# GreenleafLab/NucleoATAC

Measured on AMD Instinct MI355X. Metric: Mbp/s through occ+nuc signal pipeline, higher is better.
Workload: dtype f64

## Files before the change

nucleoatac_amd/csrc/natac_api.hip:

```cpp
#include "../../include/natac.h"
#ifndef NATAC_GNBL
#define NATAC_GNBL 2
#endif
#include "natac_kernels.hpp"
#include "natac_fft_bg.hpp"
#include "natac_occ_fast.hpp"
#include "natac_cand.hpp"
#include "natac_covsweep.hpp"
#include "natac_textz.hpp"
#include "natac_cores.hpp"
#include "natac_writer.hpp"
#include "natac_tabix.hpp"
#include "natac_pack.hpp"
#include "natac_bam.hpp"
#include "natac_bam_dev.hpp"
#include "natac_fragfile.hpp"
#include "natac_fragfile_dev.hpp"
#include "natac_fasta.hpp"
#include "natac_fuzzfit.hpp"
#include "natac_bedtab.hpp"
#include "natac_runtime.hpp"
#include "natac_pwmfit.hpp"
#include "natac_sites.hpp"
#include "natac_cellcounts.hpp"
// ... 138 lines not shown
template <int STEP>
static void occ_fast_launch(const OccFastLaunch &f) {
    natac_batch *b = f.b;
    occ_gsum_launch<STEP>(f);
    auto kd = (f.of.flags & 2) ? (f.rn16 ? natac_occ_decide<STEP, 16, true> : natac_occ_decide<STEP, 4, true>)
                               : (f.rn16 ? natac_occ_decide<STEP, 16, false> : natac_occ_decide<STEP, 4, false>);
    const bool heavy_first = b->ctx->occ_ordered;
    hipLaunchKernelGGL(kd, dim3((b->n_tiles_occ + (heavy_first ? HEAVY_CAP : 0) + 3) / 4), dim3(256), f.lds_od, b->ctx->stream, f.ct, b->d_tiles_occ,
                       b->n_tiles_occ, b->d_ranges_occ, heavy_first ? b->d_order_occ : nullptr, f.of, b->d_blk_off, b->total_blocks, b->d_gsum, b->d_grid[0], b->d_grid[1], b->d_grid[2], b->d_defer,
                       b->d_defer + 1);
}

extern "C" {

int natac_abi_version(void) { return NATAC_ABI_VERSION; }
const char *natac_last_error(void) { return g_err.c_str(); }

int natac_device_count(int *count) {
    if (!count) return fail(NATAC_E_ARG, "count is NULL");
    int n = 0;
    hipError_t e = hipGetDeviceCount(&n);
    if (e != hipSuccess) {
        *count = 0;
        return fail(NATAC_E_HIP, "hipGetDeviceCount: %s", hipGetErrorString(e));
    }
    *count = n;
    return NATAC_OK;
}

int natac_ctx_create(int device_id, natac_ctx **out) {
    if (!out) return fail(NATAC_E_ARG, "out is NULL");
    *out = nullptr;
    int n = 0;
    HIPCHK(hipGetDeviceCount(&n));
    if (device_id < 0 || device_id >= n) return fail(NATAC_E_ARG, "device %d out of range (%d devices)", device_id, n);
    HIPCHK(hipSetDevice(device_id));
    natac_ctx *c = new natac_ctx();
    c->device = device_id;
    HIPCHK(hipGetDeviceProperties(&c->prop, device_id));
    HIPCHK(hipStreamCreateWithFlags(&c->stream, hipStreamNonBlocking));
    HIPCHK(hipEventCreate(&c->t0));
    HIPCHK(hipEventCreate(&c->t1));
    {
        const char *e = getenv("NATAC_BG_DIRECT");
        c->bg_direct = e && e[0] == '1';
        e = getenv("NATAC_BG_EXT");
        c->bg_ext = !(e && e[0] == '0');
        e = getenv("NATAC_OCC_GENERAL");
        c->occ_force_general = e && e[0] == '1';
        e = getenv("NATAC_OCC_ORDER");
        c->occ_ordered = !(e && e[0] == '0');
        e = getenv("NATAC_SMOOTH_FUSED");
        c->smooth_fused = !(e && e[0] == '0');
    }
    *out = c;
    return NATAC_OK;
}

void natac_ctx_destroy(natac_ctx *c) {
    if (!c) return;
    (void)hipSetDevice(c->device);
    (void)sync_all(c);
    prof_collect(c);
    if (c->t0) (void)hipEventDestroy(c->t0);
    if (c->t1) (void)hipEventDestroy(c->t1);
    if (c->ck_stream) (void)hipStreamDestroy(c->ck_stream);
    if (c->ck_start) (void)hipEventDestroy(c->ck_start);
    if (c->d_ck) (void)hipFree(c->d_ck);
    if (c->copy_stream) (void)hipStreamDestroy(c->copy_stream);
    if (c->stream) (void)hipStreamDestroy(c->stream);
    delete c;
}

int natac_ctx_sync(natac_ctx *c) {
    if (!c) return fail(NATAC_E_ARG, "ctx is NULL");
    HIPCHK(hipSetDevice(c->device));
    HIPCHK(sync_all(c));
    prof_collect(c);
    return NATAC_OK;
}

int natac_ctx_device_info(natac_ctx *c, char *name, size_t name_len, int *n_cu, size_t *mem_bytes) {
    if (!c) return fail(NATAC_E_ARG, "ctx is NULL");
    if (name && name_len) {
        snprintf(name, name_len, "%s (%s)", c->prop.name, c->prop.gcnArchName);
    }
    if (n_cu) *n_cu = c->prop.multiProcessorCount;
    if (mem_bytes) *mem_bytes = c->prop.totalGlobalMem;
    return NATAC_OK;
}

int natac_ctx_device_ids(natac_ctx *c, int *hip_device, char *pci_bus_id, size_t pci_len) {
    if (!c) return fail(NATAC_E_ARG, "ctx is NULL");
    if (hip_device) *hip_device = c->device;
    if (pci_bus_id && pci_len) {
        pci_bus_id[0] = 0;
        HIPCHK(hipDeviceGetPCIBusId(pci_bus_id, (int)pci_len, c->device));
    }
    return NATAC_OK;
}

int natac_set_vmat(natac_ctx *c, const double *mat, int lower, int upper, int w) {
    if (!c || !mat) return fail(NATAC_E_ARG, "null argument");
    if (lower < 0 || upper <= lower || w < 0) return fail(NATAC_E_ARG, "bad vmat geometry lower=%d upper=%d w=%d", lower, upper, w);
    HIPCHK(hipSetDevice(c->device));
    HIPCHK(sync_all(c));
// ... 1126 lines not shown
    for (int64_t k = 0; k < n_cand; ++k) var[k] = var[k] * cov_reads(reads[(size_t)k]);
    return NATAC_OK;
}

static bool peaks_smooth_arm(const natac_batch *b, int order) {
    return order >= 1 && order <= 255 && peaks_plan(b->max_len, order).forms_smooth;
}

static int run_peaks_impl(natac_batch *b, const double *sig_a, const double *sig_b, bool with_stats, double min_signal, int sep,
                          int boundary, int order, const double *jitter, int64_t n_jitter, int64_t *n_cand, bool form_smooth = false) {
    if (!b || !jitter || !n_cand) return fail(NATAC_E_ARG, "null argument");
    natac_ctx *c = b->ctx;
    if (order < 1 || order > 255 || sep < 1 || boundary < 0) return fail(NATAC_E_ARG, "bad peak parameters");
    const int maxL = b->max_len;
    if (n_jitter < maxL) return fail(NATAC_E_ARG, "jitter stream (%lld) shorter than the longest chunk (%d)", (long long)n_jitter, maxL);
    HIPCHK(hipSetDevice(c->device));
    HIPCHK(sync_all(c));
    int rc;
    if (with_stats && (rc = ensure_srow(c))) return rc;
    if (!b->d_jitter || b->n_jitter < maxL) {
        if ((rc = dev_upload(c, b->d_jitter, jitter, (size_t)maxL))) return rc;
        HIPCHK(hipStreamSynchronize(c->stream));
        b->n_jitter = maxL;
    } else {
        HIPCHK(hipMemcpyAsync(b->d_jitter, jitter, (size_t)maxL * sizeof(double), hipMemcpyHostToDevice, c->stream));
        HIPCHK(hipStreamSynchronize(c->stream));
    }
    if (b->pk_order != order) {
        std::vector<long long> cap((size_t)b->nc + 1, 0);
        for (int i = 0; i < b->nc; ++i) cap[i + 1] = cap[i] + b->h_len[i] / (order + 1) + 2;
        b->slot_total = cap[b->nc];
        b->d_cap_off.reset(); b->d_slot.reset();
        if ((rc = dev_upload(c, b->d_cap_off, cap.data(), (size_t)b->nc + 1))) return rc;
        HIPCHK(hipStreamSynchronize(c->stream));
        if ((rc = dev_alloc(b->d_slot, (size_t)b->slot_total))) return rc;
        b->pk_order = order;
    }
    if (!b->d_pk_count && (rc = dev_alloc(b->d_pk_count, (size_t)b->nc))) return rc;
    if (!b->d_pk_offs && (rc = dev_alloc(b->d_pk_offs, (size_t)b->nc + 1))) return rc;
    if (form_smooth &&
        (rc = ensure_window(c, c->d_win_nuc, &c->win_nuc_M, &c->win_nuc_sd, b->out.smooth_M, b->out.smooth_sd, &c->win_nuc_sum))) return rc;
    const PeakPlan plan = peaks_plan(maxL, order);
    PeakSearch s{sig_a, sig_b, b->d_jitter, min_signal, boundary, order, sep, b->d_cap_off, b->d_slot, b->d_pk_count, b->d_status,
                 b->d_pk_offs, c->d_win_nuc, c->win_nuc_sum, form_smooth ? b->d_track[NATAC_T_SMOOTH].get() : nullptr};
    if (plan.global_lists) {
        if (b->d_pk_big.size() < (size_t)b->slot_total * 2 + 2 && (rc = dev_alloc(b->d_pk_big, (size_t)b->slot_total * 2 + 2))) return rc;
        s.big_sig = b->d_pk_big;
        s.big_pos = (int *)(b->d_pk_big + b->slot_total);
        s.big_state = (unsigned char *)(s.big_pos + b->slot_total);
    }
    natac_ctx::Ev ev;
    prof_begin(c, NATAC_K_CAND, ev);
    const ChunkTable ct = make_table(b);
    if ((rc = peaks_enqueue(plan, ct, b->nc, s, c->stream))) return rc;
    long long total = 0;
    HIPCHK(hipGetLastError());
    if (form_smooth) b->out.track[NATAC_T_SMOOTH] = TS_RUN;
    HIPCHK(hipMemcpyAsync(&total, b->d_pk_offs + b->nc, sizeof(long long), hipMemcpyDeviceToHost, c->stream));
    HIPCHK(hipStreamSynchronize(c->stream));
    if (total > b->pk_cap) {
        b->d_pk_chunk.reset(); b->d_pk_pos.reset(); b->d_pk_out.reset();
        b->pk_cap = 0;
        const long long cap = total + total / 4 + 16;
        if ((rc = dev_alloc(b->d_pk_chunk, (size_t)cap)) || (rc = dev_alloc(b->d_pk_pos, (size_t)cap)) ||
            (rc = dev_alloc(b->d_pk_out, (size_t)3 * cap))) {
            b->d_pk_chunk.reset(); b->d_pk_pos.reset();
            return rc;
        }
        b->pk_cap = cap;
    }
    if (total > 0) {
        hipLaunchKernelGGL(natac_compact_candidates, dim3((b->nc + 3) / 4), dim3(256), 0, c->stream, b->nc, b->d_pk_count, b->d_pk_offs,
                           b->d_cap_off, b->d_slot, b->d_pk_chunk, b->d_pk_pos);
        if (with_stats) {
            const VMatDev vm = make_vmat(c);
            launch_candidates(c, ct, vm, b->d_pk_chunk, b->d_pk_pos, total, b->d_track[NATAC_T_NUC_COV], b->d_track[NATAC_T_NORM],
                              b->out.bg_gen == c->model_gen ? b->d_bnum : nullptr, b->out.bg_gen == c->model_gen ? b->d_bcov : nullptr,
                              b->d_pk_out, b->d_pk_out + b->pk_cap, b->d_pk_out + 2 * b->pk_cap,
                              b->ranges256_w == c->vw ? b->d_tile256_first : nullptr, b->ranges256_w == c->vw ? b->d_ranges256 : nullptr);
        }
    }
    b->pk_has_stats = with_stats;
    prof_end(c, ev);
    HIPCHK(hipGetLastError());
    b->pk_n = total;
    *n_cand = total;
    return NATAC_OK;
}

int natac_peaks_plan(int32_t max_len, int32_t order, int32_t *kernel, int32_t *bt, int32_t *nj, int32_t *mask, int32_t *global_lists,
                     int32_t *forms_smooth, int32_t *pk_cap, int64_t *lds_bytes) {
    if (!kernel || !bt || !nj || !mask || !global_lists || !forms_smooth || !pk_cap || !lds_bytes) return fail(NATAC_E_ARG, "null argument");
    if (max_len < 1 || order < 1 || order > 255) return fail(NATAC_E_ARG, "natac_peaks_plan: a positive length and an order in 1..255");
    const PeakPlan p = peaks_plan(max_len, order);
    *kernel = p.kernel; *bt = p.bt; *nj = p.nj; *mask = p.mask; *global_lists = p.global_lists; *forms_smooth = p.forms_smooth;
    *pk_cap = p.pk_cap;
    lds_bytes[0] = (int64_t)p.lds; lds_bytes[1] = (int64_t)p.lds_smooth;
    return NATAC_OK;
}

int natac_run_peaks(natac_batch *b, double min_signal, int sep, int boundary, int order, const double *jitter, int64_t n_jitter,
                    int64_t *n_cand) {
    if (!b) return fail(NATAC_E_ARG, "batch is NULL");
    int rc;
    const bool form_smooth = b->out.track[NATAC_T_SMOOTH] == TS_PENDING && peaks_smooth_arm(b, order);
    if ((!form_smooth && (rc = need_track(b, NATAC_T_SMOOTH))) || (rc = need_candidate_inputs(b)) ||
        (rc = need_nuc_geometry(b, "natac_run_peaks"))) return rc;
// ... 201 lines not shown
```

nucleoatac_amd/csrc/natac_peaks.hpp:

```cpp
#pragma once
#include "natac_kernels.hpp"
#include "natac_runtime.hpp"

#include <utility>

namespace natac {

constexpr int PEAK_MAX = 2048;
constexpr int PK_SM_H = 30;

constexpr int PK_REG_MAX_NJ = 16;
constexpr int PK_REG1K_MIN_NJ = 256 * PK_REG_MAX_NJ / 1024 + 1;
constexpr int PK_REG_MAX_LDS = 150 * 1024;
constexpr int PK_SEG = 4096;
constexpr int PK_LIST_MIN = 2 * 128;

__host__ __device__ constexpr int peaks_list_cap(int maxL, int order) {
    const int m = maxL / (order + 1) + 2;
    return ((m < PEAK_MAX ? m : PEAK_MAX) + 7) & ~7;
}
__host__ __device__ constexpr int peaks_list_region(int pk_cap) { return pk_cap * (int)(sizeof(double) + sizeof(int) + 1); }
__host__ __device__ constexpr int peaks_wave_stride(int region, int nw) { return (region / nw) & ~7; }
__host__ __device__ constexpr bool peaks_masks_in_registers(int stride, int nj) { return stride < nj * 8; }
__host__ __device__ constexpr bool peaks_two_phase(int stride, int nj, int order) { return order > 2 && stride >= nj * 8 + PK_LIST_MIN; }
enum PeakKernel : int { PK_KERNEL_REG = 0, PK_KERNEL_SEG = 1 };
enum PeakMask : int { PK_MASK_NONE = -1, PK_MASK_REGISTERS = 0, PK_MASK_TWO_PHASE = 1, PK_MASK_DIRECT = 2 };
__host__ __device__ constexpr PeakMask peaks_mask_mode(int stride, int nj, int order) {
    return peaks_masks_in_registers(stride, nj) ? PK_MASK_REGISTERS : peaks_two_phase(stride, nj, order) ? PK_MASK_TWO_PHASE : PK_MASK_DIRECT;
}
__host__ __device__ constexpr int peaks_reg_ysn(int bt_nj, int order, bool smooth) {
    return (bt_nj + ((smooth && 2 * PK_SM_H > 2 * order + 1) ? 2 * PK_SM_H : 2 * order + 1)) & ~1;
}

struct PeakPlan {
    PeakKernel kernel;
    int bt, nj, pk_cap;
    PeakMask mask;
    bool global_lists;
    bool forms_smooth;
    size_t lds, lds_smooth;
};

__host__ __device__ constexpr PeakPlan peaks_plan(int maxL, int order) {
    PeakPlan p{};
    p.pk_cap = peaks_list_cap(maxL, order);
    const int region = peaks_list_region(p.pk_cap);
    p.bt = maxL <= 256 * PK_REG_MAX_NJ ? 256 : 1024;
    p.nj = (maxL - 1) / p.bt + 1;
    if (p.nj <= PK_REG_MAX_NJ) p.lds = (size_t)peaks_reg_ysn(p.bt * p.nj, order, false) * sizeof(double) + region;
    if (p.nj <= PK_REG_MAX_NJ && (p.bt == 256 || p.lds <= (size_t)PK_REG_MAX_LDS)) {
        p.kernel = PK_KERNEL_REG;
        p.mask = peaks_mask_mode(peaks_wave_stride(region, p.bt / 64), p.nj, order);
        p.forms_smooth = p.bt == 256 && p.mask != PK_MASK_REGISTERS;
        p.lds_smooth = p.forms_smooth ? (size_t)peaks_reg_ysn(p.bt * p.nj, order, true) * sizeof(double) + region : p.lds;
    } else {
        p.kernel = PK_KERNEL_SEG;
        p.bt = 256;
        p.nj = 0;
        p.mask = PK_MASK_NONE;
        p.global_lists = maxL / (order + 1) + 2 > p.pk_cap;
        p.lds = p.lds_smooth = (size_t)((PK_SEG + 2 * order + 1) & ~1) * sizeof(double) + region;
    }
    return p;
}
static_assert(peaks_plan(4096, 12).bt == 256 && peaks_plan(4096, 12).nj == PK_REG_MAX_NJ && peaks_plan(4096, 12).forms_smooth &&
              peaks_plan(4097, 12).bt == 1024 && peaks_plan(4097, 12).nj == PK_REG1K_MIN_NJ && !peaks_plan(4097, 12).forms_smooth &&
              peaks_plan(16384, 12).kernel == PK_KERNEL_REG && peaks_plan(16385, 12).kernel == PK_KERNEL_SEG &&
              peaks_plan(4096, 150).mask == PK_MASK_REGISTERS && !peaks_plan(4096, 150).forms_smooth, "peak search plan");

__device__ __forceinline__ void peaks_thin_and_write(int n, int pk_cap, int sep, const double *sig, const int *pos, unsigned char *state,
                                                      int *wave_cnt, int *__restrict__ dst, int *__restrict__ count_out,
                                                      int *__restrict__ status_out) {
    const int wave = threadIdx.x >> 6, lane = threadIdx.x & 63, bt = blockDim.x, nw = bt >> 6;
    const bool overflow = n > pk_cap;
    if (overflow) n = pk_cap;
    for (;;) {
        int nfree = 0;
        for (int i = threadIdx.x; i < n; i += bt) {
            if (state[i] != 0) continue;
            const double si = sig[i];
            const int pi = pos[i];
            bool top = true;
            for (int k = i - 1; top && k >= 0 && pi - pos[k] < sep; --k) top = !(state[k] <= 1 && sig[k] > si);
            for (int k = i + 1; top && k < n && pos[k] - pi < sep; ++k) top = !(state[k] <= 1 && sig[k] >= si);
            if (top) state[i] = 1; else ++nfree;
        }
        __syncthreads();
        for (int i = threadIdx.x; i < n; i += bt) {
            if (state[i] != 0) continue;
            const int pi = pos[i];
            bool ex = false;
            for (int k = i - 1; !ex && k >= 0 && pi - pos[k] < sep; --k) ex = state[k] == 1;
            for (int k = i + 1; !ex && k < n && pos[k] - pi < sep; ++k) ex = state[k] == 1;
            if (ex) { state[i] = 2; --nfree; }
        }
        if (__syncthreads_or(nfree > 0) == 0) break;
    }
    int m_out = 0;
    for (int base = 0; base < n; base += bt) {
        const int i = base + threadIdx.x;
        const bool kp = i < n && state[i] == 1;
        const unsigned long long m = __ballot(kp);
        if (lane == 0) wave_cnt[wave] = __popcll(m);
        __syncthreads();
        int off = m_out;
        int tot = 0;
        for (int w = 0; w < nw; ++w) { const int cw = wave_cnt[w]; off += (w < wave) ? cw : 0; tot += cw; }
        if (kp) dst[off + __popcll(m & ((1ull << lane) - 1ull))] = pos[i];
        m_out += tot;
        __syncthreads();
    }
    if (threadIdx.x == 0) {
        *count_out = m_out;
        if (overflow) atomicOr(status_out, 2);
    }
}

__global__ void __launch_bounds__(256) natac_peaks_chunk(ChunkTable ct, const double *__restrict__ norm,
                                                           const double *__restrict__ smooth, const double *__restrict__ jitter,
                                                           double min_signal, int boundary, int order, int sep, int seg, int pk_cap,
                                                           const long long *__restrict__ cap_off, int *__restrict__ cand_slot,
                                                           int *__restrict__ count, int *__restrict__ status,
                                                           double *__restrict__ big_sig, int *__restrict__ big_pos,
                                                           unsigned char *__restrict__ big_state) {
    extern __shared__ __attribute__((aligned(16))) double smem[];
    __shared__ double red[4];
    __shared__ int wave_cnt[16];
    __shared__ int row_cnt[4 * 16];
    const int ysn = (seg + 2 * order + 1) & ~1;
    double *ys = smem;
    double *sig = ys + ysn;
    int *pos = (int *)(sig + pk_cap);
    unsigned char *state = (unsigned char *)(pos + pk_cap);
    const int chunk = blockIdx.x;
    {
        const long long c0 = cap_off[chunk];
        const int cap_c = (int)(cap_off[chunk + 1] - c0);
        if (big_sig && cap_c > pk_cap) { sig = big_sig + c0; pos = big_pos + c0; state = big_state + c0; pk_cap = cap_c; }
    }
    const int L = ct.chunk_len[chunk];
    const long long ob = ct.out_off[chunk];
    const int wave = threadIdx.x >> 6, lane = threadIdx.x & 63;
    double mn = __builtin_inf();
    for (int g0 = threadIdx.x; g0 < L; g0 += 8 * 256) {
        double v[8];
#pragma unroll
        for (int q = 0; q < 8; ++q) {
            const int g = g0 + 256 * q;
            v[q] = __builtin_nan("");
            if (g < L) v[q] = smooth ? norm[ob + g] + smooth[ob + g] : norm[ob + g];
        }
#pragma unroll
        for (int q = 0; q < 8; ++q)
            if (v[q] == v[q]) mn = fmin(mn, v[q]);
    }
    mn = wave_min(mn);
    if (lane == 0) red[wave] = mn;
    __syncthreads();
    const double fillv = fmin(fmin(red[0], red[1]), fmin(red[2], red[3]));
    if (fillv == __builtin_inf()) {
        if (threadIdx.x == 0) count[chunk] = 0;
        return;
    }
    int n = 0;
    for (int x0 = 0; x0 < L; x0 += seg) {
        const int len = min(seg, L - x0);
        __syncthreads();
        for (int u0 = threadIdx.x; u0 < len + 2 * order; u0 += 8 * 256) {
            double v[8], jt[8];
#pragma unroll
            for (int q = 0; q < 8; ++q) {
                const int u = u0 + 256 * q;
                int g = x0 - order + u;
                g = g < 0 ? 0 : (g > L - 1 ? L - 1 : g);
                v[q] = smooth ? norm[ob + g] + smooth[ob + g] : norm[ob + g];
                jt[q] = jitter[g];
            }
#pragma unroll
            for (int q = 0; q < 8; ++q) {
                const int u = u0 + 256 * q;
                if (u < len + 2 * order) ys[u] = ((v[q] != v[q]) ? fillv : v[q]) * (1 + jt[q]);
            }
        }
        __syncthreads();
        unsigned pkf = 0;
#pragma unroll
        for (int it = 0; it < 16; ++it) {
            const int t = 256 * it + threadIdx.x;
            bool pk = t < len;
            if (pk) {
                const double y = ys[t + order];
                for (int sft = 1; sft <= order && pk; ++sft) pk = (y > ys[t + order + sft]) && (y > ys[t + order - sft]);
            }
            pkf |= pk ? (1u << it) : 0u;
        }
        double v[16];
#pragma unroll
        for (int it = 0; it < 16; ++it) {
            const int g = x0 + 256 * it + threadIdx.x;
            v[it] = 0.0;
            if (pkf & (1u << it)) v[it] = smooth ? norm[ob + g] + smooth[ob + g] : norm[ob + g];
        }
        unsigned long long bal[16];
#pragma unroll
        for (int it = 0; it < 16; ++it) {
            const int g = x0 + 256 * it + threadIdx.x;
            if (v[it] != v[it]) v[it] = fillv;
            const bool pk = (pkf & (1u << it)) && (v[it] >= min_signal) && (g >= boundary) && (g < L - boundary);
            bal[it] = __ballot(pk);
            if (lane == 0) row_cnt[it * 4 + wave] = __popcll(bal[it]);
        }
        __syncthreads();
#pragma unroll
        for (int it = 0; it < 16; ++it) {
            int off = n;
#pragma unroll
            for (int w = 0; w < 4; ++w) {
                const int cw = row_cnt[it * 4 + w];
                off += (w < wave) ? cw : 0;
                n += cw;
            }
            if ((bal[it] >> lane) & 1ull) {
                const int i = off + __popcll(bal[it] & ((1ull << lane) - 1ull));
                if (i < pk_cap) { pos[i] = x0 + 256 * it + threadIdx.x; sig[i] = v[it]; state[i] = 0; }
            }
        }
    }
    __syncthreads();
    peaks_thin_and_write(n, pk_cap, sep, sig, pos, state, wave_cnt, cand_slot + cap_off[chunk], count + chunk, status + chunk);
}

template <int NJ, int BT, bool SMOOTH = false>
__global__ void __launch_bounds__(BT) natac_peaks_chunk_reg(ChunkTable ct, const double *__restrict__ norm,
                                                               const double *__restrict__ smooth, const double *__restrict__ jitter,
                                                               double min_signal, int boundary, int order, int sep, int pk_cap,
                                                               const long long *__restrict__ cap_off, int *__restrict__ cand_slot,
                                                               int *__restrict__ count, int *__restrict__ status,
                                                               const double *__restrict__ win, double win_sum,
                                                               double *__restrict__ smooth_out) {
    extern __shared__ __attribute__((aligned(16))) double smem[];
    constexpr int NW = BT / 64;
    __shared__ double red[NW];
    __shared__ int wave_cnt[16];
    __shared__ int row_cnt[NW * NJ];
    const int ysn = peaks_reg_ysn(BT * NJ, order, SMOOTH);
    double *ys = smem;
    double *sig = ys + ysn;
    int *pos = (int *)(sig + pk_cap);
    unsigned char *state = (unsigned char *)(pos + pk_cap);
    const int chunk = blockIdx.x;
    const int L = ct.chunk_len[chunk];
    const long long ob = ct.out_off[chunk];
    const int wave = threadIdx.x >> 6, lane = threadIdx.x & 63;
    double v[NJ], jt[NJ];
    if constexpr (SMOOTH) {
        constexpr int H = PK_SM_H, M = 2 * H + 1;
        static_assert(BT >= 2 * H && M < 64, "the halo is zeroed by one pass of the workgroup; a window's validity bits fit one word");
        __shared__ unsigned long long okb[NW * NJ + 2];
        double *xs = smem;
#pragma unroll
        for (int j = 0; j < NJ; ++j) {
            const int g = threadIdx.x + BT * j;
            double x = __builtin_nan("");
            if (g < L) x = norm[ob + g];
            v[j] = x;
            const bool okv = x == x;
            xs[H + g] = okv ? (x < 0 ? 0.0 : x) : 0.0;
            const unsigned long long m = __ballot(okv);
            if (lane == 0) okb[1 + NW * j + wave] = m;
        }
        if (threadIdx.x < 2 * H) xs[threadIdx.x < H ? threadIdx.x : BT * NJ + threadIdx.x] = 0.0;
        if (threadIdx.x == 0) { okb[0] = 0ull; okb[NW * NJ + 1] = 0ull; }
        __syncthreads();
        const int g0 = threadIdx.x * NJ;
        double num[NJ];
#pragma unroll
        for (int o = 0; o < NJ; ++o) num[o] = 0.0;
        if (g0 < L) {
#pragma unroll
            for (int kk = 0; kk < 2 * H + NJ; ++kk) {
                const int k = 2 * H + NJ - 1 - kk;
                const double r = xs[g0 + k];
#pragma unroll
                for (int o = 0; o < NJ; ++o) {
                    const int n = o + 2 * H - k;
                    if (n >= 0 && n < M) num[o] = fma(win[n], r, num[o]);
                }
            }
        }
        __syncthreads();
        if (g0 < L) {
#pragma unroll
            for (int o = 0; o < NJ; ++o) xs[g0 + o] = num[o];
        }
        __syncthreads();
#pragma unroll
        for (int j = 0; j < NJ; ++j) {
            const int g = threadIdx.x + BT * j;
            const bool in = g < L;
            jt[j] = 0.0;
            if (in) jt[j] = jitter[g];
            double den = win_sum;
            const int iw = NW * j + wave;
            constexpr unsigned long long HM = (1ull << H) - 1ull;
            const bool clean = (okb[iw] >> (64 - H)) == HM && okb[iw + 1] == ~0ull && (okb[iw + 2] & HM) == HM;
            if (__ballot(!clean) != 0ull) {
                constexpr unsigned long long FULL = (1ull << M) - 1ull;
                const int p = g - H + 64, i = p >> 6, sh = p & 63;
                unsigned long long f = okb[i] >> sh;
                if (sh) f |= okb[i + 1] << (64 - sh);
                f &= FULL;
                bool generic = false;
                if (in && f != FULL) {
                    const int lo = __builtin_ctzll(f | (1ull << M)), hi = __builtin_clzll(f | 1ull) - (64 - M);
                    if (f == 0ull) den = 0.0;
                    else if (f == ((FULL >> lo) << lo)) den = win[M + 2 * H - lo];
                    else if (f == (FULL >> hi)) den = win[2 * M + hi];
                    else generic = true;
                }
                if (__ballot(generic) != 0ull) {
                    double d = 0.0;
#pragma unroll 8
                    for (int n = 0; n < M; ++n) {
                        const double wv = win[n];
                        if ((f >> (2 * H - n)) & 1ull) d = fma(wv, 1.0, d);
                    }
                    if (generic) den = d;
                }
            }
            if (in) {
                const double s = (den == 0.0) ? __builtin_nan("") : xs[g] / den;
                smooth_out[ob + g] = s;
                v[j] += s;
            }
        }
    } else {
#pragma unroll
    for (int j = 0; j < NJ; ++j) {
        const int g = threadIdx.x + BT * j;
        v[j] = __builtin_nan("");
        jt[j] = 0.0;
        if (g < L) {
            v[j] = smooth ? norm[ob + g] + smooth[ob + g] : norm[ob + g];
            jt[j] = jitter[g];
        }
    }
    }
    double mn = __builtin_inf();
#pragma unroll
    for (int j = 0; j < NJ; ++j)
        if (v[j] == v[j]) mn = fmin(mn, v[j]);
    mn = wave_min(mn);
    if (lane == 0) red[wave] = mn;
    __syncthreads();
    double fillv = red[0];
#pragma unroll
    for (int w = 1; w < NW; ++w) fillv = fmin(fillv, red[w]);
    if (fillv == __builtin_inf()) {
        if (threadIdx.x == 0) count[chunk] = 0;
        return;
    }
#pragma unroll
    for (int j = 0; j < NJ; ++j) {
        const int g = threadIdx.x + BT * j;
        if (v[j] != v[j]) v[j] = fillv;
        if (g < L) {
            const double y = v[j] * (1 + jt[j]);
            ys[order + g] = y;
            if (g == 0)
                for (int u = 0; u < order; ++u) ys[u] = y;
            if (g == L - 1)
                for (int u = 0; u < order; ++u) ys[order + L + u] = y;
        }
    }
    __syncthreads();
    unsigned long long bal[NJ];
    {
        const int stride = peaks_wave_stride(peaks_list_region(pk_cap), NW);
        unsigned long long *wmask = (unsigned long long *)((unsigned char *)sig + wave * stride);
        unsigned short *wlist = (unsigned short *)(wmask + NJ);
        const int cap = (stride - NJ * 8) / 2;
        const bool two_phase = peaks_two_phase(stride, NJ, order);
        if (peaks_masks_in_registers(stride, NJ)) {
#pragma unroll
            for (int j = 0; j < NJ; ++j) {
                const int g = threadIdx.x + BT * j;
                bool pk = g < L && (v[j] >= min_signal) && (g >= boundary) && (g < L - boundary);
                if (pk) {
                    const double y = ys[g + order];
                    for (int sft = 1; sft <= order && pk; ++sft) pk = (y > ys[g + order + sft]) && (y > ys[g + order - sft]);
                }
                bal[j] = __ballot(pk);
                if (lane == 0) row_cnt[j * NW + wave] = __popcll(bal[j]);
            }
        } else {
        if (lane < NJ) wmask[lane] = 0ull;
        __builtin_amdgcn_wave_barrier();
        int cnt = 0;
        const int o1 = order < 2 ? order : 2;
#pragma unroll
        for (int j = 0; j < NJ; ++j) {
            const int g = threadIdx.x + BT * j;
            bool pk = g < L && (v[j] >= min_signal) && (g >= boundary) && (g < L - boundary);
            double y = 0.0;
            if (pk) {
                y = ys[g + order];
                for (int sft = 1; sft <= o1 && pk; ++sft) pk = (y > ys[g + order + sft]) && (y > ys[g + order - sft]);
            }
            const unsigned long long m = __ballot(pk);
            const int alive = __popcll(m);
            if (two_phase && cnt + alive <= cap) {
                if (pk) wlist[cnt + __builtin_amdgcn_mbcnt_hi((unsigned)(m >> 32), __builtin_amdgcn_mbcnt_lo((unsigned)m, 0u))] =
                            (unsigned short)(j * 64 + lane);
                cnt += alive;
            } else {
                if (pk)
                    for (int sft = o1 + 1; sft <= order && pk; ++sft) pk = (y > ys[g + order + sft]) && (y > ys[g + order - sft]);
                const unsigned long long mf = __ballot(pk);
                if (lane == 0) wmask[j] = mf;
            }
        }
        __builtin_amdgcn_wave_barrier();
        unsigned int *wm32 = (unsigned int *)wmask;
        for (int idx = lane; idx - lane < cnt; idx += 64) {
            if (idx < cnt) {
                const int e = wlist[idx], jj = e >> 6, ll = e & 63;
                const int g = (wave << 6) + ll + BT * jj;
                const double y = ys[g + order];
                bool pk = true;
                for (int sft = 3; sft <= order && pk; ++sft) pk = (y > ys[g + order + sft]) && (y > ys[g + order - sft]);
                if (pk) atomicOr(&wm32[2 * jj + (ll >> 5)], 1u << (ll & 31));
            }
        }
        __builtin_amdgcn_wave_barrier();
#pragma unroll
        for (int j = 0; j < NJ; ++j) {
            bal[j] = wmask[j];
            if (lane == 0) row_cnt[j * NW + wave] = __popcll(bal[j]);
        }
        }
    }
    __syncthreads();
    int n = 0;
#pragma unroll
    for (int j = 0; j < NJ; ++j) {
        int off = n;
#pragma unroll
        for (int w = 0; w < NW; ++w) {
            const int cw = row_cnt[j * NW + w];
            off += (w < wave) ? cw : 0;
            n += cw;
        }
        if ((bal[j] >> lane) & 1ull) {
            const int i = off + __popcll(bal[j] & ((1ull << lane) - 1ull));
            if (i < pk_cap) { pos[i] = threadIdx.x + BT * j; sig[i] = v[j]; state[i] = 0; }
        }
    }
    __syncthreads();
    peaks_thin_and_write(n, pk_cap, sep, sig, pos, state, wave_cnt, cand_slot + cap_off[chunk], count + chunk, status + chunk);
}

__global__ void __launch_bounds__(1024) natac_scan_counts(const int *__restrict__ count, int nc, long long *__restrict__ offs) {
    __shared__ long long wtot[16];
    const int t = threadIdx.x, lane = t & 63, wave = t >> 6;
    long long carry = 0;
    for (int base = 0; base < nc; base += 4096) {
        const int i0 = base + 4 * t;
        int c[4];
#pragma unroll
        for (int q = 0; q < 4; ++q) c[q] = (i0 + q < nc) ? count[i0 + q] : 0;
        const long long mine = (long long)c[0] + c[1] + c[2] + c[3];
        long long incl = mine;
#pragma unroll
        for (int d = 1; d < 64; d <<= 1) {
            const long long up = __shfl_up(incl, d);
            if (lane >= d) incl += up;
        }
        if (lane == 63) wtot[wave] = incl;
        __syncthreads();
        long long before = carry, total = 0;
#pragma unroll
        for (int w = 0; w < 16; ++w) {
            const long long v = wtot[w];
            before += (w < wave) ? v : 0;
            total += v;
        }
        long long run = before + incl - mine;
#pragma unroll
        for (int q = 0; q < 4; ++q) {
            if (i0 + q < nc) offs[i0 + q] = run;
            run += c[q];
        }
        carry += total;
        __syncthreads();
    }
    if (t == 0) offs[nc] = carry;
}

__global__ void __launch_bounds__(256) natac_compact_candidates(int nc, const int *__restrict__ count,
                                                                  const long long *__restrict__ offs,
                                                                  const long long *__restrict__ cap_off,
                                                                  const int *__restrict__ cand_slot, int *__restrict__ cand_chunk,
                                                                  int *__restrict__ cand_pos) {
    const int chunk = blockIdx.x * 4 + (threadIdx.x >> 6);
    if (chunk >= nc) return;
    const int lane = threadIdx.x & 63;
    const int n = count[chunk];
    const long long o = offs[chunk];
    const int *src = cand_slot + cap_off[chunk];
    for (int i = lane; i < n; i += 64) { cand_chunk[o + i] = chunk; cand_pos[o + i] = src[i]; }
}

// ... 28 lines not shown
        if (threadIdx.x == 0) total_s = 0;
        __syncthreads();
        const int f0 = lower_bound_i32(cen, 0, nfr, p - flank);
        const int f1 = lower_bound_i32(cen, f0, nfr, p + flank + 1);
        int mine = 0;
        for (int f = f0 + threadIdx.x; f < f1; f += 256) {
            const int n = iln[f];
            if (n >= 0 && n < U) { atomicAdd(&hist_s[n], 1); ++mine; }
        }
        if (mine) atomicAdd(&total_s, mine);
        __syncthreads();
        const double tot = (double)total_s;
        for (int q = 0; q < nj && q < 4; ++q) {
            const int j = threadIdx.x + 256 * q;
            if (j < U) nd[q] = nd[q] + (double)hist_s[j] / tot;
        }
        __syncthreads();
    }
    for (int q = 0; q < nj && q < 4; ++q) {
        const int j = threadIdx.x + 256 * q;
        if (j < U) nuc_dist[(long long)chunk * U + j] = nd[q];
    }
}

using PeaksRegFn = decltype(&natac_peaks_chunk_reg<1, 256, false>);
template <int BT, bool SMOOTH, int NJ0, int... I>
static PeaksRegFn peaks_reg_instance(int nj, std::integer_sequence<int, I...>) {
    static const PeaksRegFn table[] = {natac_peaks_chunk_reg<NJ0 + I, BT, SMOOTH>...};
    return table[nj - NJ0];
}
static PeaksRegFn peaks_reg_kernel(int bt, int nj, bool smooth) {
    using At256 = std::make_integer_sequence<int, PK_REG_MAX_NJ>;
    using At1024 = std::make_integer_sequence<int, PK_REG_MAX_NJ - PK_REG1K_MIN_NJ + 1>;
    if (bt == 256) return smooth ? peaks_reg_instance<256, true, 1>(nj, At256{}) : peaks_reg_instance<256, false, 1>(nj, At256{});
    return peaks_reg_instance<1024, false, PK_REG1K_MIN_NJ>(nj, At1024{});
}

struct PeakSearch {
    const double *norm, *smooth;
    const double *jitter;
    double min_signal;
    int boundary, order, sep;
    const long long *cap_off;
    int *slot, *count, *status;
    long long *offs;
    const double *win;
    double win_sum;
    double *smooth_out;
    double *big_sig;
    int *big_pos;
    unsigned char *big_state;
};

static int peaks_enqueue(const PeakPlan &p, const ChunkTable &ct, int nc, const PeakSearch &s, hipStream_t st) {
    hipLaunchKernelGGL(natac_status_clear, dim3((nc + 255) / 256), dim3(256), 0, st, s.status, nc, 2);
    if (p.kernel == PK_KERNEL_REG) {
        const bool form_smooth = s.smooth_out != nullptr;
        if (form_smooth && !p.forms_smooth) return fail(NATAC_E_STATE, "peak search: this arm cannot form the smoothed track");
        const size_t lds = form_smooth ? p.lds_smooth : p.lds;
        const PeaksRegFn kfn = peaks_reg_kernel(p.bt, p.nj, form_smooth);
        if (lds > 64 * 1024) HIPCHK(hipFuncSetAttribute((const void *)kfn, hipFuncAttributeMaxDynamicSharedMemorySize, (int)lds));
        hipLaunchKernelGGL(kfn, dim3(nc), dim3(p.bt), lds, st, ct, s.norm, form_smooth ? nullptr : s.smooth, s.jitter, s.min_signal,
                           s.boundary, s.order, s.sep, p.pk_cap, s.cap_off, s.slot, s.count, s.status, s.win, s.win_sum, s.smooth_out);
    } else {
        hipLaunchKernelGGL(natac_peaks_chunk, dim3(nc), dim3(p.bt), p.lds, st, ct, s.norm, s.smooth, s.jitter, s.min_signal, s.boundary,
                           s.order, s.sep, PK_SEG, p.pk_cap, s.cap_off, s.slot, s.count, s.status, s.big_sig, s.big_pos, s.big_state);
    }
    hipLaunchKernelGGL(natac_scan_counts, dim3(1), dim3(1024), 0, st, s.count, nc, s.offs);
    return NATAC_OK;
}

}
```

nucleoatac_amd/csrc/natac_runtime.hpp:

```cpp
#pragma once
#include "../../include/natac.h"
#include "natac_textz.hpp"

#include <algorithm>
#include <cstdarg>
#include <cstdio>
#include <cstdlib>
#include <map>
#include <mutex>
#include <string>
#include <unordered_map>
#include <utility>
#include <vector>

static thread_local std::string g_err;

static int fail(int code, const char *fmt, ...) {
    char buf[512];
    va_list ap;
    va_start(ap, fmt);
    vsnprintf(buf, sizeof buf, fmt, ap);
    va_end(ap);
    g_err = buf;
    return code;
// ... 12 lines not shown

template <class T>
class PoolBuf {
  public:
    PoolBuf() = default;
    PoolBuf(PoolBuf &&o) noexcept : p_(o.p_), n_(o.n_) { o.p_ = nullptr; o.n_ = 0; }
    PoolBuf &operator=(PoolBuf &&o) noexcept {
        if (this != &o) { reset(); p_ = o.p_; n_ = o.n_; o.p_ = nullptr; o.n_ = 0; }
        return *this;
    }
    ~PoolBuf() { reset(); }
    void reset() { dev_free(p_); p_ = nullptr; n_ = 0; }
    hipError_t alloc(size_t n) {
        reset();
        if (n == 0) n = 1;
        void *p = nullptr;
        const hipError_t e = pool_alloc(&p, n * sizeof(T));
        if (e == hipSuccess) { p_ = (T *)p; n_ = n; }
        return e;
    }
    T *get() const { return p_; }
    operator T *() const { return p_; }
    size_t size() const { return n_; }

  private:
    T *p_ = nullptr;
    size_t n_ = 0;
};

template <class T>
static int dev_alloc(PoolBuf<T> &buf, size_t n) {
    HIPCHK(buf.alloc(n));
    return NATAC_OK;
}

struct natac_ctx {
    int device = 0;
    hipStream_t stream = nullptr;
    hipStream_t copy_stream = nullptr;
    hipDeviceProp_t prop;
    PoolBuf<double> d_vmat, d_vmat_pad, d_srow, d_sizes;
    PoolBuf<double> d_lrt;
    long long lrt_gen = -1;
    PoolBuf<double> d_ctab;
    long long ctab_gen = -1;
    int vlower = 0, vupper = 0, vw = 0, R = 0, W = 0, sizes_upper = 0;
    bool have_vmat = false, have_sizes = false, srow_dirty = true;
    bool vmat_zero = false, srow_zero = false;
    long long model_gen = 0;
    PoolBuf<double> d_fft_tw, d_fft_k;
    PoolBuf<double> d_fft_mtab, d_fft_swt;
    bool smooth_fused = true;
    bool bg_ext = true;
    bool fft_dirty = true, bg_direct = false, occ_ordered = true, occ_zero_nfr = false;
    std::vector<double> h_sizes;
    PoolBuf<double> d_nucp, d_nfrp, d_alphas;
    int occ_upper = 0, n_alpha = 0, step = 0, halfstep = 0, flank = 0;
    double cutoff = 0;
    bool have_occ = false;
    int occ_zero_flags = 0;
    PoolBuf<double> d_occ_q4, d_occ_rho;
    int occ_nm = 0;
    bool occ_fast_ok = false, occ_force_general = false, occ_rn16 = false;
    double occ_b_floor = 0;
    PoolBuf<double> d_win_nuc, d_win_occ;
    PoolBuf<double> d_wb_occ;
    int wb_M = 0, wb_step = 0;
    int win_nuc_M = 0, win_occ_M = 0;
    double win_nuc_sd = -1, win_occ_sd = -1;
    double win_nuc_sum = 0, win_occ_sum = 0;
    bool profiling = false;
    struct Ev { int k; hipEvent_t a, b; hipStream_t st; };
    std::vector<Ev> pending;
    double prof_ms[NATAC_K_COUNT] = {0};
    int64_t prof_n[NATAC_K_COUNT] = {0};
    hipEvent_t t0 = nullptr, t1 = nullptr;
    hipStream_t ck_stream = nullptr;
    hipEvent_t ck_start = nullptr;
    long long *d_ck = nullptr;
    int ck_cap = 0;
    bool ck_active = false;
    struct Iv { int k; float t0, t1; };
    std::vector<Iv> ck_iv;
    PoolBuf<natac_text::P10> d_p10;
    PoolBuf<natac_deflate::CrcTables> d_crc;
};

enum TrackState : unsigned char { TS_EMPTY = 0, TS_PENDING, TS_RUN , TS_HOST  };
struct BatchOutputs {
    TrackState track[NATAC_T_COUNT] = {};
    bool grids = false;
    long long bg_gen = -1;
    int nuc_w = -1, nuc_lower = -1, nuc_upper = -1;
    bool occ_cov_by_nuc = false;
    int smooth_M = 0;
    double smooth_sd = 0;
    int occ_step = -1, occ_half = -1, occ_flank = -1, occ_upper = -1;
};

struct natac_batch {
    natac_ctx *ctx = nullptr;
    int nc = 0, max_len = 0;
    long long nf = 0, nb = 0, total_bp = 0, total_grid = 0;
    int bias_left = 0, bias_right = 0;
    std::vector<int> h_len;
    std::vector<long long> h_out_off, h_grid_off;
// ... 267 lines not shown
```

Measured before the change: 3622.

## Make peak-search kernels persistent with residency-sized grid and next-chunk prefetch

```diff
diff --git a/nucleoatac_amd/csrc/natac_api.hip b/nucleoatac_amd/csrc/natac_api.hip
--- a/nucleoatac_amd/csrc/natac_api.hip
+++ b/nucleoatac_amd/csrc/natac_api.hip
@@ -214,6 +214,8 @@
         c->occ_ordered = !(e && e[0] == '0');
         e = getenv("NATAC_SMOOTH_FUSED");
         c->smooth_fused = !(e && e[0] == '0');
+        e = getenv("NATAC_PEAKS_GRID");
+        c->peaks_grid_cap = e ? atoi(e) : 0;
     }
     *out = c;
     return NATAC_OK;
@@ -1446,7 +1448,7 @@
     natac_ctx::Ev ev;
     prof_begin(c, NATAC_K_CAND, ev);
     const ChunkTable ct = make_table(b);
-    if ((rc = peaks_enqueue(plan, ct, b->nc, s, c->stream))) return rc;
+    if ((rc = peaks_enqueue(plan, ct, b->nc, s, c->prop.multiProcessorCount, c->peaks_grid_cap, c->stream))) return rc;
     long long total = 0;
     HIPCHK(hipGetLastError());
     if (form_smooth) b->out.track[NATAC_T_SMOOTH] = TS_RUN;
diff --git a/nucleoatac_amd/csrc/natac_peaks.hpp b/nucleoatac_amd/csrc/natac_peaks.hpp
--- a/nucleoatac_amd/csrc/natac_peaks.hpp
+++ b/nucleoatac_amd/csrc/natac_peaks.hpp
@@ -39,7 +39,25 @@
     bool global_lists;
     bool forms_smooth;
     size_t lds, lds_smooth;
+    int wg_cu, wg_cu_smooth;
 };
+
+constexpr int PK_CU_LDS = 160 * 1024;
+constexpr int PK_CU_WAVES = 32;
+constexpr int PK_SIMD_VGPRS = 512;
+constexpr int PK_SEG_WAVES = 4;
+constexpr int PK_STATIC_LDS = 1536;
+__host__ __device__ constexpr int peaks_reg_vgprs(int nj, bool prefetch) { return (40 + 4 * nj + (prefetch ? 2 * nj : 0) + 7) & ~7; }
+__host__ __device__ constexpr int peaks_reg_waves(int bt, int nj, bool prefetch) {
+    const int w = PK_SIMD_VGPRS / peaks_reg_vgprs(nj, prefetch);
+    return bt == 1024 ? 4 : (w < PK_CU_WAVES / 4 ? w : PK_CU_WAVES / 4);
+}
+__host__ __device__ constexpr int peaks_resident(int bt, size_t lds, int waves_simd) {
+    const int by_lds = (int)((size_t)PK_CU_LDS / (lds + PK_STATIC_LDS));
+    const int by_regs = waves_simd * 4 / (bt / 64);
+    const int r = by_lds < by_regs ? by_lds : by_regs;
+    return r < 1 ? 1 : r;
+}
 
 __host__ __device__ constexpr PeakPlan peaks_plan(int maxL, int order) {
     PeakPlan p{};
@@ -53,6 +71,8 @@
         p.mask = peaks_mask_mode(peaks_wave_stride(region, p.bt / 64), p.nj, order);
         p.forms_smooth = p.bt == 256 && p.mask != PK_MASK_REGISTERS;
         p.lds_smooth = p.forms_smooth ? (size_t)peaks_reg_ysn(p.bt * p.nj, order, true) * sizeof(double) + region : p.lds;
+        p.wg_cu = peaks_resident(p.bt, p.lds, peaks_reg_waves(p.bt, p.nj, false));
+        p.wg_cu_smooth = p.forms_smooth ? peaks_resident(p.bt, p.lds_smooth, peaks_reg_waves(p.bt, p.nj, true)) : p.wg_cu;
     } else {
         p.kernel = PK_KERNEL_SEG;
         p.bt = 256;
@@ -60,6 +80,7 @@
         p.mask = PK_MASK_NONE;
         p.global_lists = maxL / (order + 1) + 2 > p.pk_cap;
         p.lds = p.lds_smooth = (size_t)((PK_SEG + 2 * order + 1) & ~1) * sizeof(double) + region;
+        p.wg_cu = p.wg_cu_smooth = peaks_resident(p.bt, p.lds, PK_SEG_WAVES);
     }
     return p;
 }
@@ -67,16 +88,18 @@
               peaks_plan(4097, 12).bt == 1024 && peaks_plan(4097, 12).nj == PK_REG1K_MIN_NJ && !peaks_plan(4097, 12).forms_smooth &&
               peaks_plan(16384, 12).kernel == PK_KERNEL_REG && peaks_plan(16385, 12).kernel == PK_KERNEL_SEG &&
               peaks_plan(4096, 150).mask == PK_MASK_REGISTERS && !peaks_plan(4096, 150).forms_smooth, "peak search plan");
-
-__device__ __forceinline__ void peaks_thin_and_write(int n, int pk_cap, int sep, const double *sig, const int *pos, unsigned char *state,
+static_assert(peaks_plan(2120, 12).wg_cu == 6 && peaks_plan(2120, 12).wg_cu_smooth == 5 && peaks_plan(400, 12).wg_cu_smooth == 8 &&
+              peaks_plan(16384, 12).wg_cu == 1 && peaks_plan(4097, 12).wg_cu == 1 && peaks_plan(16385, 12).wg_cu == 3, "peak search residency");
+
+__device__ __forceinline__ void peaks_thin_and_write(int tid, int n, int pk_cap, int sep, const double *sig, const int *pos, unsigned char *state,
                                                       int *wave_cnt, int *__restrict__ dst, int *__restrict__ count_out,
                                                       int *__restrict__ status_out) {
-    const int wave = threadIdx.x >> 6, lane = threadIdx.x & 63, bt = blockDim.x, nw = bt >> 6;
+    const int wave = tid >> 6, lane = tid & 63, bt = blockDim.x, nw = bt >> 6;
     const bool overflow = n > pk_cap;
     if (overflow) n = pk_cap;
     for (;;) {
         int nfree = 0;
-        for (int i = threadIdx.x; i < n; i += bt) {
+        for (int i = tid; i < n; i += bt) {
             if (state[i] != 0) continue;
             const double si = sig[i];
             const int pi = pos[i];
@@ -86,7 +109,7 @@
             if (top) state[i] = 1; else ++nfree;
         }
         __syncthreads();
-        for (int i = threadIdx.x; i < n; i += bt) {
+        for (int i = tid; i < n; i += bt) {
             if (state[i] != 0) continue;
             const int pi = pos[i];
             bool ex = false;
@@ -98,7 +121,7 @@
     }
     int m_out = 0;
     for (int base = 0; base < n; base += bt) {
-        const int i = base + threadIdx.x;
+        const int i = base + tid;
         const bool kp = i < n && state[i] == 1;
         const unsigned long long m = __ballot(kp);
         if (lane == 0) wave_cnt[wave] = __popcll(m);
@@ -110,13 +133,13 @@
         m_out += tot;
         __syncthreads();
     }
-    if (threadIdx.x == 0) {
+    if (tid == 0) {
         *count_out = m_out;
         if (overflow) atomicOr(status_out, 2);
     }
 }
 
-__global__ void __launch_bounds__(256) natac_peaks_chunk(ChunkTable ct, const double *__restrict__ norm,
+__global__ void __launch_bounds__(256, PK_SEG_WAVES) natac_peaks_chunk(ChunkTable ct, int nc, const double *__restrict__ norm,
                                                            const double *__restrict__ smooth, const double *__restrict__ jitter,
                                                            double min_signal, int boundary, int order, int sep, int seg, int pk_cap,
                                                            const long long *__restrict__ cap_off, int *__restrict__ cand_slot,
@@ -129,10 +152,16 @@
     __shared__ int row_cnt[4 * 16];
     const int ysn = (seg + 2 * order + 1) & ~1;
     double *ys = smem;
+    const int lds_cap = pk_cap;
+    for (int chunk = blockIdx.x; chunk < nc; chunk += gridDim.x) {
+    __syncthreads();
+    int tid = threadIdx.x;
+    asm volatile("" : "+v"(tid));
+    asm volatile("" : "+s"(order), "+s"(sep), "+s"(boundary), "+s"(seg));
     double *sig = ys + ysn;
-    int *pos = (int *)(sig + pk_cap);
-    unsigned char *state = (unsigned char *)(pos + pk_cap);
-    const int chunk = blockIdx.x;
+    int *pos = (int *)(sig + lds_cap);
+    unsigned char *state = (unsigned char *)(pos + lds_cap);
+    pk_cap = lds_cap;
     {
         const long long c0 = cap_off[chunk];
         const int cap_c = (int)(cap_off[chunk + 1] - c0);
@@ -140,9 +169,9 @@
     }
     const int L = ct.chunk_len[chunk];
     const long long ob = ct.out_off[chunk];
-    const int wave = threadIdx.x >> 6, lane = threadIdx.x & 63;
+    const int wave = tid >> 6, lane = tid & 63;
     double mn = __builtin_inf();
-    for (int g0 = threadIdx.x; g0 < L; g0 += 8 * 256) {
+    for (int g0 = tid; g0 < L; g0 += 8 * 256) {
         double v[8];
 #pragma unroll
         for (int q = 0; q < 8; ++q) {
@@ -159,14 +188,14 @@
     __syncthreads();
     const double fillv = fmin(fmin(red[0], red[1]), fmin(red[2], red[3]));
     if (fillv == __builtin_inf()) {
-        if (threadIdx.x == 0) count[chunk] = 0;
-        return;
+        if (tid == 0) count[chunk] = 0;
+        continue;
     }
     int n = 0;
     for (int x0 = 0; x0 < L; x0 += seg) {
         const int len = min(seg, L - x0);
         __syncthreads();
-        for (int u0 = threadIdx.x; u0 < len + 2 * order; u0 += 8 * 256) {
+        for (int u0 = tid; u0 < len + 2 * order; u0 += 8 * 256) {
             double v[8], jt[8];
 #pragma unroll
             for (int q = 0; q < 8; ++q) {
@@ -186,7 +215,7 @@
         unsigned pkf = 0;
 #pragma unroll
         for (int it = 0; it < 16; ++it) {
-            const int t = 256 * it + threadIdx.x;
+            const int t = 256 * it + tid;
             bool pk = t < len;
             if (pk) {
                 const double y = ys[t + order];
@@ -197,14 +226,14 @@
         double v[16];
 #pragma unroll
         for (int it = 0; it < 16; ++it) {
-            const int g = x0 + 256 * it + threadIdx.x;
+            const int g = x0 + 256 * it + tid;
             v[it] = 0.0;
             if (pkf & (1u << it)) v[it] = smooth ? norm[ob + g] + smooth[ob + g] : norm[ob + g];
         }
         unsigned long long bal[16];
 #pragma unroll
         for (int it = 0; it < 16; ++it) {
-            const int g = x0 + 256 * it + threadIdx.x;
+            const int g = x0 + 256 * it + tid;
             if (v[it] != v[it]) v[it] = fillv;
             const bool pk = (pkf & (1u << it)) && (v[it] >= min_signal) && (g >= boundary) && (g < L - boundary);
             bal[it] = __ballot(pk);
@@ -222,16 +251,17 @@
             }
             if ((bal[it] >> lane) & 1ull) {
                 const int i = off + __popcll(bal[it] & ((1ull << lane) - 1ull));
-                if (i < pk_cap) { pos[i] = x0 + 256 * it + threadIdx.x; sig[i] = v[it]; state[i] = 0; }
-            }
-        }
-    }
-    __syncthreads();
-    peaks_thin_and_write(n, pk_cap, sep, sig, pos, state, wave_cnt, cand_slot + cap_off[chunk], count + chunk, status + chunk);
+                if (i < pk_cap) { pos[i] = x0 + 256 * it + tid; sig[i] = v[it]; state[i] = 0; }
+            }
+        }
+    }
+    __syncthreads();
+    peaks_thin_and_write(tid, n, pk_cap, sep, sig, pos, state, wave_cnt, cand_slot + cap_off[chunk], count + chunk, status + chunk);
+    }
 }
 
 template <int NJ, int BT, bool SMOOTH = false>
-__global__ void __launch_bounds__(BT) natac_peaks_chunk_reg(ChunkTable ct, const double *__restrict__ norm,
+__global__ void __launch_bounds__(BT, peaks_reg_waves(BT, NJ, SMOOTH)) natac_peaks_chunk_reg(ChunkTable ct, int nc, const double *__restrict__ norm,
                                                                const double *__restrict__ smooth, const double *__restrict__ jitter,
                                                                double min_signal, int boundary, int order, int sep, int pk_cap,
                                                                const long long *__restrict__ cap_off, int *__restrict__ cand_slot,
@@ -248,10 +278,28 @@
     double *sig = ys + ysn;
     int *pos = (int *)(sig + pk_cap);
     unsigned char *state = (unsigned char *)(pos + pk_cap);
-    const int chunk = blockIdx.x;
-    const int L = ct.chunk_len[chunk];
-    const long long ob = ct.out_off[chunk];
-    const int wave = threadIdx.x >> 6, lane = threadIdx.x & 63;
+    const int stride_c = (int)gridDim.x;
+    [[maybe_unused]] double nx[SMOOTH ? NJ : 1];
+    [[maybe_unused]] int L1 = 0, L2 = 0;
+    [[maybe_unused]] long long ob1 = 0, ob2 = 0;
+    if constexpr (SMOOTH) {
+        if ((int)blockIdx.x < nc) { L1 = ct.chunk_len[blockIdx.x]; ob1 = ct.out_off[blockIdx.x]; }
+        if ((int)blockIdx.x + stride_c < nc) { L2 = ct.chunk_len[blockIdx.x + stride_c]; ob2 = ct.out_off[blockIdx.x + stride_c]; }
+#pragma unroll
+        for (int j = 0; j < NJ; ++j) {
+            const int g = threadIdx.x + BT * j;
+            nx[j] = __builtin_nan("");
+            if (g < L1) nx[j] = norm[ob1 + g];
+        }
+    }
+    for (int chunk = blockIdx.x; chunk < nc; chunk += stride_c) {
+    __syncthreads();
+    int tid = threadIdx.x;
+    asm volatile("" : "+v"(tid));
+    asm volatile("" : "+s"(order), "+s"(pk_cap), "+s"(sep), "+s"(boundary));
+    const int wave = tid >> 6, lane = tid & 63;
+    const int L = SMOOTH ? L1 : ct.chunk_len[chunk];
+    const long long ob = SMOOTH ? ob1 : ct.out_off[chunk];
     double v[NJ], jt[NJ];
     if constexpr (SMOOTH) {
         constexpr int H = PK_SM_H, M = 2 * H + 1;
@@ -260,19 +308,26 @@
         double *xs = smem;
 #pragma unroll
         for (int j = 0; j < NJ; ++j) {
-            const int g = threadIdx.x + BT * j;
-            double x = __builtin_nan("");
-            if (g < L) x = norm[ob + g];
+            const int g = tid + BT * j;
+            const double x = nx[j];
             v[j] = x;
             const bool okv = x == x;
             xs[H + g] = okv ? (x < 0 ? 0.0 : x) : 0.0;
             const unsigned long long m = __ballot(okv);
             if (lane == 0) okb[1 + NW * j + wave] = m;
         }
-        if (threadIdx.x < 2 * H) xs[threadIdx.x < H ? threadIdx.x : BT * NJ + threadIdx.x] = 0.0;
-        if (threadIdx.x == 0) { okb[0] = 0ull; okb[NW * NJ + 1] = 0ull; }
-        __syncthreads();
-        const int g0 = threadIdx.x * NJ;
+        if (tid < 2 * H) xs[tid < H ? tid : BT * NJ + tid] = 0.0;
+        if (tid == 0) { okb[0] = 0ull; okb[NW * NJ + 1] = 0ull; }
+        L1 = L2; ob1 = ob2; L2 = 0;
+        if ((long long)chunk + 2 * stride_c < nc) { L2 = ct.chunk_len[chunk + 2 * stride_c]; ob2 = ct.out_off[chunk + 2 * stride_c]; }
+#pragma unroll
+        for (int j = 0; j < NJ; ++j) {
+            const int g = tid + BT * j;
+            nx[j] = __builtin_nan("");
+            if (g < L1) nx[j] = norm[ob1 + g];
+        }
+        __syncthreads();
+        const int g0 = tid * NJ;
         double num[NJ];
 #pragma unroll
         for (int o = 0; o < NJ; ++o) num[o] = 0.0;
@@ -296,7 +351,7 @@
         __syncthreads();
 #pragma unroll
         for (int j = 0; j < NJ; ++j) {
-            const int g = threadIdx.x + BT * j;
+            const int g = tid + BT * j;
             const bool in = g < L;
             jt[j] = 0.0;
             if (in) jt[j] = jitter[g];
@@ -337,7 +392,7 @@
     } else {
 #pragma unroll
     for (int j = 0; j < NJ; ++j) {
-        const int g = threadIdx.x + BT * j;
+        const int g = tid + BT * j;
         v[j] = __builtin_nan("");
         jt[j] = 0.0;
         if (g < L) {
@@ -357,12 +412,12 @@
 #pragma unroll
     for (int w = 1; w < NW; ++w) fillv = fmin(fillv, red[w]);
     if (fillv == __builtin_inf()) {
-        if (threadIdx.x == 0) count[chunk] = 0;
-        return;
+        if (tid == 0) count[chunk] = 0;
+        continue;
     }
 #pragma unroll
     for (int j = 0; j < NJ; ++j) {
-        const int g = threadIdx.x + BT * j;
+        const int g = tid + BT * j;
         if (v[j] != v[j]) v[j] = fillv;
         if (g < L) {
             const double y = v[j] * (1 + jt[j]);
@@ -384,7 +439,7 @@
         if (peaks_masks_in_registers(stride, NJ)) {
 #pragma unroll
             for (int j = 0; j < NJ; ++j) {
-                const int g = threadIdx.x + BT * j;
+                const int g = tid + BT * j;
                 bool pk = g < L && (v[j] >= min_signal) && (g >= boundary) && (g < L - boundary);
                 if (pk) {
                     const double y = ys[g + order];
@@ -400,7 +455,7 @@
         const int o1 = order < 2 ? order : 2;
 #pragma unroll
         for (int j = 0; j < NJ; ++j) {
-            const int g = threadIdx.x + BT * j;
+            const int g = tid + BT * j;
             bool pk = g < L && (v[j] >= min_signal) && (g >= boundary) && (g < L - boundary);
             double y = 0.0;
             if (pk) {
@@ -453,11 +508,12 @@
         }
         if ((bal[j] >> lane) & 1ull) {
             const int i = off + __popcll(bal[j] & ((1ull << lane) - 1ull));
-            if (i < pk_cap) { pos[i] = threadIdx.x + BT * j; sig[i] = v[j]; state[i] = 0; }
-        }
-    }
-    __syncthreads();
-    peaks_thin_and_write(n, pk_cap, sep, sig, pos, state, wave_cnt, cand_slot + cap_off[chunk], count + chunk, status + chunk);
+            if (i < pk_cap) { pos[i] = tid + BT * j; sig[i] = v[j]; state[i] = 0; }
+        }
+    }
+    __syncthreads();
+    peaks_thin_and_write(tid, n, pk_cap, sep, sig, pos, state, wave_cnt, cand_slot + cap_off[chunk], count + chunk, status + chunk);
+    }
 }
 
 __global__ void __launch_bounds__(1024) natac_scan_counts(const int *__restrict__ count, int nc, long long *__restrict__ offs) {
@@ -592,19 +648,24 @@
     unsigned char *big_state;
 };
 
-static int peaks_enqueue(const PeakPlan &p, const ChunkTable &ct, int nc, const PeakSearch &s, hipStream_t st) {
+static int peaks_enqueue(const PeakPlan &p, const ChunkTable &ct, int nc, const PeakSearch &s, int n_cu, int grid_cap, hipStream_t st) {
     hipLaunchKernelGGL(natac_status_clear, dim3((nc + 255) / 256), dim3(256), 0, st, s.status, nc, 2);
+    const bool form_smooth = p.kernel == PK_KERNEL_REG && s.smooth_out != nullptr;
+    long long grid = (long long)(n_cu > 0 ? n_cu : 1) * (form_smooth ? p.wg_cu_smooth : p.wg_cu);
+    if (grid_cap > 0 && grid > grid_cap) grid = grid_cap;
+    if (grid > nc) grid = nc;
     if (p.kernel == PK_KERNEL_REG) {
-        const bool form_smooth = s.smooth_out != nullptr;
         if (form_smooth && !p.forms_smooth) return fail(NATAC_E_STATE, "peak search: this arm cannot form the smoothed track");
         const size_t lds = form_smooth ? p.lds_smooth : p.lds;
         const PeaksRegFn kfn = peaks_reg_kernel(p.bt, p.nj, form_smooth);
         if (lds > 64 * 1024) HIPCHK(hipFuncSetAttribute((const void *)kfn, hipFuncAttributeMaxDynamicSharedMemorySize, (int)lds));
-        hipLaunchKernelGGL(kfn, dim3(nc), dim3(p.bt), lds, st, ct, s.norm, form_smooth ? nullptr : s.smooth, s.jitter, s.min_signal,
-                           s.boundary, s.order, s.sep, p.pk_cap, s.cap_off, s.slot, s.count, s.status, s.win, s.win_sum, s.smooth_out);
+        hipLaunchKernelGGL(kfn, dim3((unsigned)grid), dim3(p.bt), lds, st, ct, nc, s.norm, form_smooth ? nullptr : s.smooth, s.jitter,
+                           s.min_signal, s.boundary, s.order, s.sep, p.pk_cap, s.cap_off, s.slot, s.count, s.status, s.win, s.win_sum,
+                           s.smooth_out);
     } else {
-        hipLaunchKernelGGL(natac_peaks_chunk, dim3(nc), dim3(p.bt), p.lds, st, ct, s.norm, s.smooth, s.jitter, s.min_signal, s.boundary,
-                           s.order, s.sep, PK_SEG, p.pk_cap, s.cap_off, s.slot, s.count, s.status, s.big_sig, s.big_pos, s.big_state);
+        hipLaunchKernelGGL(natac_peaks_chunk, dim3((unsigned)grid), dim3(p.bt), p.lds, st, ct, nc, s.norm, s.smooth, s.jitter, s.min_signal,
+                           s.boundary, s.order, s.sep, PK_SEG, p.pk_cap, s.cap_off, s.slot, s.count, s.status, s.big_sig, s.big_pos,
+                           s.big_state);
     }
     hipLaunchKernelGGL(natac_scan_counts, dim3(1), dim3(1024), 0, st, s.count, nc, s.offs);
     return NATAC_OK;
diff --git a/nucleoatac_amd/csrc/natac_runtime.hpp b/nucleoatac_amd/csrc/natac_runtime.hpp
--- a/nucleoatac_amd/csrc/natac_runtime.hpp
+++ b/nucleoatac_amd/csrc/natac_runtime.hpp
@@ -88,6 +88,7 @@
     PoolBuf<double> d_fft_mtab, d_fft_swt;
     bool smooth_fused = true;
     bool bg_ext = true;
+    int peaks_grid_cap = 0;
     bool fft_dirty = true, bg_direct = false, occ_ordered = true, occ_zero_nfr = false;
     std::vector<double> h_sizes;
     PoolBuf<double> d_nucp, d_nfrp, d_alphas;
```

New measurement: 3580. 1.2% lower.
